# Fil/nd4js

Hardware: AMD Instinct MI355X
Metric: fp64 GFLOP/s: matmul N=4096 & SVD N=2048; % of MFMA/HBM peak (higher is better)
Workload: dtype f64

## Files before the change

nd4js_amd/build.py:

```python
import os
import shutil
import subprocess
import sys
from concurrent.futures import ThreadPoolExecutor

HERE = os.path.dirname(os.path.abspath(__file__))
CSRC = os.path.join(HERE, "csrc")
OBJ = os.path.join(CSRC, "_obj")
LIB = os.path.join(HERE, "libnd4hip.so")
ADDON = os.path.join(HERE, "js", "nd4hip_napi.node")
ARCH = "gfx950"
HIP_SOURCES = ["nd4hip_core.hip", "nd4hip_api.hip", "nd4hip_host.hip", "gemm.hip", "lu.hip", "qr.hip", "svd.hip", "svd_block.hip", "trsm.hip", "chol.hip", "hess.hip", "bidiag.hip", "rrqr.hip"]
HIPCC_FLAGS = ["-O3", "--offload-arch=" + ARCH, "-fPIC", "-std=c++17", "-ffp-contract=on",
               "-mllvm", "-pragma-unroll-threshold=200000", "-Wall", "-Wno-unused-function"]


def _hipcc():
    for c in (os.environ.get("HIPCC"), shutil.which("hipcc"), "/opt/rocm/bin/hipcc"):
        if c and os.path.exists(c):
            return c
    raise RuntimeError("hipcc not found (need ROCm with gfx950 support)")


def _newer(target, deps):
    if not os.path.exists(target):
        return True
    t = os.path.getmtime(target)
    return any(os.path.getmtime(d) > t for d in deps)


def build_lib(force=False, verbose=False):
    os.makedirs(OBJ, exist_ok=True)
    hipcc = _hipcc()
    headers = [os.path.join(CSRC, f) for f in os.listdir(CSRC) if f.endswith(".h")]
    headers.append(os.path.join(HERE, "..", "include", "nd4hip.h"))
    jobs = []
    for s in HIP_SOURCES:
        src = os.path.join(CSRC, s)
        obj = os.path.join(OBJ, s.replace(".hip", ".o"))
        if force or _newer(obj, [src] + headers):
            jobs.append([hipcc] + HIPCC_FLAGS + ["-c", src, "-o", obj])

    def run(cmd):
        if verbose:
            print(" ".join(cmd), flush=True)
        r = subprocess.run(cmd, stdout=subprocess.PIPE, stderr=subprocess.STDOUT, text=True)
        if r.returncode != 0:
            raise RuntimeError("hipcc failed:\n%s\n%s" % (" ".join(cmd), r.stdout))
        if verbose and r.stdout.strip():
            print(r.stdout)
    with ThreadPoolExecutor(max_workers=4) as ex:
        list(ex.map(run, jobs))
    objs = [os.path.join(OBJ, s.replace(".hip", ".o")) for s in HIP_SOURCES]
    if force or jobs or _newer(LIB, objs):
        run([hipcc, "-shared", "-fPIC", "--offload-arch=" + ARCH, "-o", LIB] + objs)
    return LIB


def build_addon(force=False, verbose=False):
    inc = "/usr/include/node"
    src = os.path.join(CSRC, "napi_shim.c")
    if not (os.path.exists(os.path.join(inc, "node_api.h")) and os.path.exists(src)):
        return None
    if force or _newer(ADDON, [src, os.path.join(HERE, "..", "include", "nd4hip.h")]):
        cmd = ["gcc", "-O2", "-fPIC", "-shared", "-std=c11", "-Wall", "-I" + inc, "-I" + os.path.join(HERE, "..", "include"),
# ... 14 lines not shown
```

nd4js_amd/csrc/bidiag.hip:

```cpp
#include "nd4hip_internal.h"
#include "xchg16.h"
#include <cstdio>
#include <cstdlib>

namespace {

constexpr int GR = 8;

__device__ __forceinline__ double blk_max(double v, double* s_red) {
  for (int off = 32; off > 0; off >>= 1) v = fmax(v, __shfl_xor(v, off));
  if ((threadIdx.x & 63) == 0) s_red[threadIdx.x >> 6] = v;
  __syncthreads();
  v = fmax(fmax(s_red[0], s_red[1]), fmax(s_red[2], s_red[3]));
  __syncthreads();
  return v;
}
__device__ __forceinline__ double blk_sum(double v, double* s_red) {
  for (int off = 32; off > 0; off >>= 1) v += __shfl_xor(v, off);
  if ((threadIdx.x & 63) == 0) s_red[threadIdx.x >> 6] = v;
  __syncthreads();
  v = (s_red[0] + s_red[1]) + (s_red[2] + s_red[3]);
  __syncthreads();
  return v;
}
// ... 650 lines not shown
      rq[3] = HpReq{A4r + (unsigned)(t * 2 + 1) * 16, true};
      rq[4] = HpReq{R4p + (unsigned)((q1 * 16 + l1 / E) * V4 + E + l1 % E) * 16, t == 0};
      hp_wait<5>(rs, rq, xv, tag, dead, X.abort, status, delay & 255);
      if (t < T) { s_y[t] = xv[0]; s_cu[t] = xv[1]; }
      if (t == 0) s_alpha = xv[4];
      const double wm = wave_max(xv[2]);
      const double f = wm > 0.0 ? xv[2] * fast_rcp(wm) : 0.0;
      const double wS = wave_sum(xv[3] * f * f);
      if (lane == 0) { s_wm[wave] = wm; s_wS[wave] = wS; }
    }
    if (dead) s_dead = 1;
    __syncthreads();
    if (s_dead) break;
    BP_STAMP(5)
#pragma unroll
    for (int ai = 0; ai < E; ai++) {
      const double ya = s_y[tr + 16 * ai];
#pragma unroll
      for (int bi = 0; bi < E; bi++) a[ai][bi] = fma(-ya, vc[bi], fma(-ur[ai], zc[bi], a[ai][bi]));
    }
    BP_STAMP(6)
  }
#undef BP_STAMP
  if (stamps && t == 0) for (int k = 0; k < 7; k++) stamps[wg * 8 + k] = tacc[k];
}

struct BdWs { double* z; double* y; double* zpart; long sV, sZ; int ncols_total; };

int reflect_left(nd4hip_handle* h, int batch, const Blk& b, const double* A2, long lda, long sA, int acol, const double* tau, long sTau, int tidx, const BdWs& ws) {
  const int nr = b.r1 - b.r0, nc = b.c1 - b.c0;
  if (nr <= 0 || nc <= 0) return 0;
  const int P = (nr + GR - 1) / GR;
  hipLaunchKernelGGL(bd_colsum, dim3((unsigned)((nc + 63) / 64), (unsigned)P, (unsigned)batch), dim3(256), 0, h->stream,
                     b, A2, lda, sA, acol, tau, sTau, tidx, ws.zpart, ws.sZ, ws.ncols_total);
  hipLaunchKernelGGL(bd_colsum_reduce, dim3((unsigned)((nc + 31) / 32), (unsigned)batch), dim3(256), 0, h->stream,
                     b.c0, b.c1, P, ws.zpart, ws.sZ, ws.ncols_total, tau, sTau, tidx, ws.z, ws.sV);
  hipLaunchKernelGGL(bd_rank1, dim3((unsigned)((nc + 255) / 256), (unsigned)((nr + 15) / 16), (unsigned)batch), dim3(256), 0, h->stream,
                     b, A2 + acol, lda, sA, ws.z, ws.sV, tau, sTau, (const int*)nullptr, 0l, tidx);
  ND4_HIP(hipGetLastError());
  return 0;
}
int reflect_right(nd4hip_handle* h, int batch, const Blk& b, const double* v, long sVR, const int* flag, long sF, int fidx, const BdWs& ws) {
  const int nr = b.r1 - b.r0, nc = b.c1 - b.c0;
  if (nr <= 0 || nc <= 0) return 0;
  hipLaunchKernelGGL(bd_rowdot, dim3((unsigned)((nr + 3) / 4), (unsigned)batch), dim3(256), 0, h->stream, b, v, sVR, 2.0, flag, sF, fidx, ws.y, ws.sV);
  hipLaunchKernelGGL(bd_rank1, dim3((unsigned)((nc + 255) / 256), (unsigned)((nr + 15) / 16), (unsigned)batch), dim3(256), 0, h->stream,
                     b, ws.y, 1l, ws.sV, v, sVR, (const double*)nullptr, 0l, flag, sF, fidx);
  ND4_HIP(hipGetLastError());
  return 0;
}

}

int nd4_gebrd(nd4hip_handle* h, int64_t batch64, int64_t M64, int64_t N64, const double* A, double* U, double* B, double* V) {
  ND4_CHECK_ARG(M64 < 32768 && N64 < 32768 && batch64 < 65536, "nd4_gebrd: extent out of range");
  const int M = (int)M64, N = (int)N64, batch = (int)batch64;
  if (M == 0 || N == 0 || batch == 0) return 0;
  const int K = M < N ? M : N, J = M >= N ? K : K + 1;
  const int mx = M > N ? M : N;
  const int Pmax = (M + GR - 1) / GR;
  Nd4WsScope scope(h);
  void* p = nullptr;
  const size_t nd = (size_t)batch * ((size_t)M * N + (size_t)M * K + (size_t)K * N + (size_t)K + 2 * (size_t)mx + (size_t)(Pmax + 24) * mx);
  ND4_TRY(nd4_ws_alloc(h, sizeof(double) * nd + sizeof(int) * (size_t)batch * (2 * (size_t)K + 2) + 256, &p));
  double* W = static_cast<double*>(p);
  double* UL = W + (size_t)batch * M * N;
  double* VR = UL + (size_t)batch * M * K;
  double* tauL = VR + (size_t)batch * K * N;
  BdWs ws;
  ws.z = tauL + (size_t)batch * K; ws.y = ws.z + (size_t)batch * mx; ws.zpart = ws.y + (size_t)batch * mx;
  ws.sV = mx; ws.sZ = (long)Pmax * mx; ws.ncols_total = mx;
  int* flagR = reinterpret_cast<int*>(ws.zpart + (size_t)batch * (Pmax + 24) * mx);
  int* flips = flagR + (size_t)batch * K + 1;
  const long sW = (long)M * N, sUL = (long)M * K, sVRm = (long)K * N;
  ND4_HIP(hipMemcpyAsync(W, A, sizeof(double) * (size_t)batch * sW, hipMemcpyDeviceToDevice, h->stream));
  ND4_HIP(hipMemsetAsync(VR, 0, sizeof(double) * (size_t)batch * sVRm, h->stream));
  ND4_HIP(hipMemsetAsync(flagR, 0, sizeof(int) * (size_t)batch * K, h->stream));

  static const bool fused_off = getenv("ND4HIP_BIDIAG_UNFUSED") != nullptr;
  const bool no_persist = getenv("ND4HIP_BIDIAG_NO_PERSIST") != nullptr;
  bool persist = !fused_off && !no_persist && batch == 1 && M >= 128 && N >= 128 && M <= 2048 && N <= 2048;
  if (persist) {
    int per_cu = 0;
    const hipError_t oe = mx <= 512 ? hipOccupancyMaxActiveBlocksPerMultiprocessor(&per_cu, bdp<2>, 256, 0)
                        : mx <= 1024 ? hipOccupancyMaxActiveBlocksPerMultiprocessor(&per_cu, bdp<4>, 256, 0)
                                     : hipOccupancyMaxActiveBlocksPerMultiprocessor(&per_cu, bdp<8>, 256, 0);
    persist = oe == hipSuccess && (long)per_cu * h->num_cu >= 256;
  }
  if (persist) {
    const int E = mx <= 512 ? 2 : (mx <= 1024 ? 4 : 8), T = 16 * E;
    const size_t V1 = 3 * T, V2 = 2 * E, V3 = T, V4 = 2 * E;
    const size_t xbytes = 16 * 2 * 256 * (V1 + V2 + V3 + V4) + (size_t)BP_NREP * (BP_REP_A2 + BP_REP_A4);
    Nd4WsScope scope2(h);
    void* qp = nullptr;
    ND4_TRY(nd4_ws_alloc(h, sizeof(double) * (size_t)K * M + xbytes + 64, &qp));
    double* ULt = static_cast<double*>(qp);
    BdPx X;
    X.base = reinterpret_cast<qx_u64*>(ULt + (size_t)K * M);
    X.o1 = 0; X.o2 = X.o1 + (unsigned)(2 * 256 * V1 * 16); X.o3 = X.o2 + (unsigned)(2 * 256 * V2 * 16); X.o4 = X.o3 + (unsigned)(2 * 256 * V3 * 16);
    X.oA2 = X.o4 + (unsigned)(2 * 256 * V4 * 16); X.oA4 = X.oA2 + BP_NREP * BP_REP_A2; X.bytes = X.oA4 + BP_NREP * BP_REP_A4;
    X.abort = reinterpret_cast<int*>(reinterpret_cast<char*>(X.base) + xbytes);
    ND4_HIP(hipMemsetAsync(X.base, 0, xbytes + 64, h->stream));
    static const bool want_stamps = getenv("ND4HIP_BDP_STAMPS") != nullptr;
    const int delay = getenv("ND4HIP_BDP_DELAY") ? atoi(getenv("ND4HIP_BDP_DELAY")) : (0 << 8 | 4);
    long long* stamps = nullptr;
    if (want_stamps) { void* sp = nullptr; ND4_TRY(nd4_ws_alloc(h, sizeof(long long) * 256 * 8, &sp)); stamps = static_cast<long long*>(sp); }
    if (E == 2) hipLaunchKernelGGL(bdp<2>, dim3(256), dim3(256), 0, h->stream, W, M, N, K, ULt, tauL, VR, flagR, X, h->xstat, delay, stamps, nd4_test_drop_panel());
// ... 38 lines not shown
      hipLaunchKernelGGL(bd2_finish_row, dim3((unsigned)((N - prev - 1 + 255) / 256)), dim3(256), 0, h->stream, W, N, prev, rowfin);
    ND4_HIP(hipGetLastError());
  } else
  for (int i = 0; i < K; i++) {
    hipLaunchKernelGGL(bd_vec_col, dim3((unsigned)batch), dim3(256), 0, h->stream, W, M, N, i, UL, K, tauL);
    {
      Blk b{W, N, sW, i, M, i + 1, N};
      ND4_TRY(reflect_left(h, batch, b, UL, K, sUL, i, tauL, K, i, ws));
    }
    if (i + 1 < N - 1) {
      hipLaunchKernelGGL(bd_vec_row, dim3((unsigned)batch), dim3(256), 0, h->stream, W, M, N, i, VR, K, flagR);
      Blk b{W, N, sW, i + 1, M, i + 1, N};
      ND4_TRY(reflect_right(h, batch, b, VR + (long)i * N, sVRm, flagR, K, i, ws));
    }
  }
  {
    const unsigned gy = (unsigned)(K < 512 ? K : 512);
    hipLaunchKernelGGL(bd_extract, dim3((unsigned)((J + 255) / 256), gy, (unsigned)batch), dim3(256), 0, h->stream, W, M, N, B, K, J);
  }
  if (batch <= 4 && K >= 256) {
    Nd4WsScope scope2(h);
    void* q = nullptr;
    ND4_TRY(nd4_ws_alloc(h, sizeof(double) * ((size_t)N * K + (size_t)N * J + (size_t)K + 16), &q));
    double* VRt = static_cast<double*>(q);
    double* Vt = VRt + (size_t)N * K;
    double* twos = Vt + (size_t)N * J;
    hipLaunchKernelGGL(bd_fill, dim3((unsigned)((K + 255) / 256)), dim3(256), 0, h->stream, twos, K, 2.0);
    for (int m = 0; m < batch; m++) {
      ND4_TRY(nd4_wy_form(h, M, K, UL + (size_t)m * sUL, tauL + (size_t)m * K, 1, U + (size_t)m * M * K, K));
      ND4_TRY(nd4_transpose(h, K, N, VR + (size_t)m * sVRm, N, VRt, K, 1, 0, 0));
      ND4_TRY(nd4_wy_form(h, N, K, VRt, twos, 1, Vt, J));
      ND4_TRY(nd4_transpose(h, N, J, Vt, J, V + (size_t)m * J * N, N, 1, 0, 0));
    }
  } else {
  {
    const unsigned gy = (unsigned)(M < 512 ? M : 512);
    hipLaunchKernelGGL(bd_set_identity, dim3((unsigned)((K + 255) / 256), gy, (unsigned)batch), dim3(256), 0, h->stream, U, M, K);
  }
  for (int i = K - 1; i >= 0; i--) {
    Blk b{U, K, (long)M * K, i, M, i, K};
    ND4_TRY(reflect_left(h, batch, b, UL, K, sUL, i, tauL, K, i, ws));
  }
  {
    const unsigned gy = (unsigned)(J < 512 ? J : 512);
    hipLaunchKernelGGL(bd_set_identity, dim3((unsigned)((N + 255) / 256), gy, (unsigned)batch), dim3(256), 0, h->stream, V, J, N);
  }
  for (int k = K - 1; k >= 0; k--) {
    if (!(k + 1 < N - 1)) continue;
    Blk b{V, N, (long)J * N, k + 1, J, k + 1, N};
    ND4_TRY(reflect_right(h, batch, b, VR + (long)k * N, sVRm, flagR, K, k, ws));
  }
  }
  ND4_HIP(hipGetLastError());
  return nd4_givens_signs(h, batch, M, K, J, M > N, U, K, (long)M * K, B, J, (long)K * J, tauL, K, flips);
}
```

nd4js_amd/csrc/nd4hip_internal.h:

```cpp
#pragma once
#include <hip/hip_runtime.h>
#include <cstdint>
#include <cstdio>
#include <cstdarg>
#include <vector>
#include "../../include/nd4hip.h"

struct Nd4WsBlock { char* p; size_t size, used; };

struct Nd4Stage { void* p; size_t bytes; bool in_use; };

struct nd4hip_handle {
  int device = 0;
  hipStream_t own_stream = nullptr;
  hipStream_t stream = nullptr;
  std::vector<Nd4WsBlock> ws;
  std::vector<Nd4Stage> stage;
  size_t stage_bytes = 0;
  void* pinned = nullptr;
  size_t pinned_bytes = 0;
  hipEvent_t ev0 = nullptr, ev1 = nullptr;
  hipEvent_t ev_order = nullptr;
  hipStream_t copy_stream = nullptr;
  hipStream_t aux_stream = nullptr;
// ... 15 lines not shown
  }
  ~Nd4DeviceGuard() { if (switched) (void)hipSetDevice(prev); }
  Nd4DeviceGuard(const Nd4DeviceGuard&) = delete;
  Nd4DeviceGuard& operator=(const Nd4DeviceGuard&) = delete;
};

struct Nd4Prof {
  nd4hip_handle* h; bool active;
  Nd4Prof(nd4hip_handle* hh, const char* op, double flops, double bytes);
  ~Nd4Prof();
  Nd4Prof(const Nd4Prof&) = delete;
  Nd4Prof& operator=(const Nd4Prof&) = delete;
};

void nd4_set_error(const char* fmt, ...);
int  nd4_xchg_check(nd4hip_handle* h, const char* where);
int  nd4_test_drop_panel();
int  nd4_hip_fail(hipError_t e, const char* what, const char* file, int line);

#define ND4_HIP(expr)                                                           \
  do { hipError_t _e = (expr);                                                  \
       if (_e != hipSuccess) return nd4_hip_fail(_e, #expr, __FILE__, __LINE__); } while (0)
#define ND4_CHECK_ARG(cond, ...)                                                \
  do { if (!(cond)) { nd4_set_error(__VA_ARGS__); return ND4HIP_ERR_ARG; } } while (0)
#define ND4_TRY(expr) do { int _rc = (expr); if (_rc != 0) return _rc; } while (0)

int nd4_ws_alloc(nd4hip_handle* h, size_t bytes, void** out);
struct Nd4WsScope {
  nd4hip_handle* h; size_t nblocks; size_t used_last; unsigned generation;
  explicit Nd4WsScope(nd4hip_handle* hh);
  ~Nd4WsScope();
};
int nd4_pinned(nd4hip_handle* h, size_t bytes, void** out);

int nd4_gemm(nd4hip_handle* h, bool transA, bool transB, int64_t M, int64_t N, int64_t K,
             double alpha, const double* A, int64_t lda, int64_t sA,
             const double* B, int64_t ldb, int64_t sB,
             double beta, double* C, int64_t ldc, int64_t sC, int64_t batch);

int nd4_getrf(nd4hip_handle* h, int64_t batch, int64_t N, const double* A, double* LU, int32_t* P);
int nd4_getrf_nopivot(nd4hip_handle* h, int64_t batch, int64_t N, const double* A, double* LU, int32_t* P);
int nd4_trsm(nd4hip_handle* h, bool upper, bool unit, int64_t batch, int64_t M, int64_t J, const double* T, int64_t sT, double* X);
int nd4_syrk_lower(nd4hip_handle* h, int64_t N, int64_t K, double alpha, const double* A, int64_t lda, int64_t sA,
                   double beta, double* C, int64_t ldc, int64_t sC, int64_t batch);
int nd4_gemm_nt_lower(nd4hip_handle* h, int64_t N, int64_t K, double alpha, const double* A, int64_t lda, int64_t sA,
                      const double* B, int64_t ldb, int64_t sB, double beta, double* C, int64_t ldc, int64_t sC, int64_t batch);
int nd4_trsm_ld(nd4hip_handle* h, bool upper, bool unit, int64_t batch, int64_t M, int64_t J, const double* T, int64_t ldT, int64_t sT,
                double* X, int64_t sX);
int nd4_trsm_t(nd4hip_handle* h, int64_t batch, int64_t M, int64_t J, const double* T, int64_t ldT, int64_t sT, double* X, int64_t sX);
int nd4_trsm_t_ex(nd4hip_handle* h, bool unit, int64_t batch, int64_t M, int64_t J, const double* T, int64_t ldT, int64_t sT, double* X, int64_t sX);
int nd4_ldltrf(nd4hip_handle* h, int64_t batch, int64_t N, const double* S, double* LD);
int nd4_ldltrs(nd4hip_handle* h, int64_t batch, int64_t N, int64_t J, const double* LD, int64_t sLD, const double* Y, int64_t sY, double* X);
int nd4_gebrd(nd4hip_handle* h, int64_t batch, int64_t M, int64_t N, const double* A, double* U, double* B, double* V);
int nd4_gehrd(nd4hip_handle* h, int64_t batch, int64_t N, const double* A, double* U, double* H);
int nd4_potrf(nd4hip_handle* h, int64_t batch, int64_t N, const double* S, double* L, int* flags);
int nd4_potrs(nd4hip_handle* h, int64_t batch, int64_t N, int64_t J, const double* L, int64_t sL, const double* Y, int64_t sY, double* X);
int nd4_qrls(nd4hip_handle* h, int64_t batch, int64_t N, int64_t M, int64_t I, int64_t J, const double* Q, int64_t sQ,
             const double* R, int64_t sR, const double* Y, int64_t sY, double* X);
int nd4_svdls(nd4hip_handle* h, int64_t batch, int64_t N, int64_t M, int64_t I, int64_t J, const double* U, int64_t sU,
              const double* sv, int64_t sSv, const double* V, int64_t sV, const double* Y, int64_t sY, double* X);
int nd4_getrs(nd4hip_handle* h, int64_t batch, int64_t N, int64_t J, const double* LU, int64_t sLU, const int32_t* P, int64_t sP,
              const double* Y, int64_t sY, double* X);
int nd4_geqrf_q(nd4hip_handle* h, int64_t batch, int64_t M, int64_t N, const double* A, double* Q, double* R);
int nd4_geqr2_panel(nd4hip_handle* h, int batch, int M, double* A, double* V, double* T);
int nd4_givens_signs(nd4hip_handle* h, int batch, int M, int L, int ncols, bool lu_rule, double* Q, long ldq, long sQ,
                     double* R, long ldr, long sR, const double* taus, long sTau, int* flips);
int nd4_wy_form(nd4hip_handle* h, int M, int n, const double* V, const double* Tdiag, int bs, double* Q, int Lq);
int nd4_geqrf_q_ex(nd4hip_handle* h, int64_t batch, int64_t M, int64_t N, const double* A, double* Q, double* R, bool full);
int nd4_geqp3(nd4hip_handle* h, int64_t batch, int64_t M, int64_t N, const double* A, double* Q, double* R, int32_t* P, bool full);
int nd4_qp3rank(nd4hip_handle* h, int64_t batch, int64_t M, int64_t N, const double* R, int64_t sR, int* rank);
int nd4_qp3ls(nd4hip_handle* h, int64_t batch, int64_t N, int64_t M, int64_t I, int64_t J, const double* Q, int64_t sQ,
              const double* R, int64_t sR, const int32_t* P, int64_t sP, const double* Y, int64_t sY, double* X, int* rank_out);
int nd4_gesvdj(nd4hip_handle* h, int64_t batch, int64_t M, int64_t N, const double* A,
               double* U, double* sv, double* V, int* sweeps_out, double* offnorm_out);

int nd4_copy_matrix(nd4hip_handle* h, int64_t rows, int64_t cols, const double* src, int64_t lds,
                    double* dst, int64_t ldd, int64_t batch, int64_t ssrc, int64_t sdst);
int nd4_transpose(nd4hip_handle* h, int64_t rows, int64_t cols, const double* src, int64_t lds,
                  double* dst, int64_t ldd, int64_t batch, int64_t ssrc, int64_t sdst);
int nd4_set_identity(nd4hip_handle* h, int64_t rows, int64_t cols, double* dst, int64_t ldd,
                     int64_t batch, int64_t sdst);
```

nd4js_amd/csrc/svd.hip:

```cpp
#include "svd_internal.h"
#include "dpp.h"
#include <cmath>
#include <cfloat>
#include <cstring>
#include <cstdlib>

namespace {

constexpr int MAX_SWEEPS = 60;

__device__ __forceinline__ double wave_sum(double v) {
#pragma unroll
  for (int off = 32; off > 0; off >>= 1) v += __shfl_xor(v, off);
  return v;
}

__global__ __launch_bounds__(256) void jac_step(double* __restrict__ Wm, double* __restrict__ Utm, int N, long strideM,
                                                 int n2, int step, double tol2, JacState* __restrict__ st,
                                                 const double* __restrict__ floor2, unsigned long long* __restrict__ offmax) {
  const int mat = blockIdx.y;
  if (st[mat].done) return;
  int p, q;
  nd4_rr_pair(n2, step, blockIdx.x, p, q);
  if (q >= N) return;
// ... 378 lines not shown
      }
      if (sweeps >= MAX_SWEEPS) break;
    }
  }
  if (padded) {
    ND4_TRY(nd4_copy_matrix(h, N, N, Wp, Np, W, N, batch, sMp, sM));
    ND4_TRY(nd4_copy_matrix(h, N, N, Utpad, Np, Ut, N, batch, sMp, sM));
  }
  (void)svrp;
  hipLaunchKernelGGL(jac_norms, dim3((unsigned)((N + 3) / 4), (unsigned)batch), dim3(256), 0, h->stream, W, N, sM, svr);
  hipLaunchKernelGGL(jac_rank, dim3((unsigned)((N + 255) / 256), (unsigned)batch), dim3(256), 0, h->stream, svr, N, rank);
  hipLaunchKernelGGL(jac_emit, dim3((unsigned)N, (unsigned)batch), dim3(256), 0, h->stream, W, Ut, N, sM, svr, rank, V, Utp, sv);
  if (N < 128) {
    hipLaunchKernelGGL(jac_complete, dim3((unsigned)batch), dim3(1024), 0, h->stream, V, N, sM, sv, floor2, scratch);
    ND4_HIP(hipGetLastError());
  } else {
    int* z0d = reinterpret_cast<int*>(scratch);
    int* z0h = reinterpret_cast<int*>(static_cast<char*>(pin) + 64);
    hipLaunchKernelGGL(jac_count_rank, dim3((unsigned)((batch + 63) / 64)), dim3(64), 0, h->stream, sv, N, floor2, z0d, batch);
    ND4_HIP(hipGetLastError());
    ND4_HIP(hipMemcpyAsync(z0h, z0d, sizeof(int) * (size_t)batch, hipMemcpyDeviceToHost, h->stream));
    ND4_HIP(hipStreamSynchronize(h->stream));
    for (int m = 0; m < batch; m++) {
      const int r = z0h[m];
      if (r >= N) continue;
      double* Vm = V + (size_t)m * sM;
      if (r == 0) { ND4_TRY(nd4_set_identity(h, N, N, Vm, N, 1, sM)); continue; }
      Nd4WsScope scope3(h);
      void* q = nullptr;
      ND4_TRY(nd4_ws_alloc(h, sizeof(double) * ((size_t)N * N + 2 * (size_t)N * r), &q));
      double* Qf = static_cast<double*>(q);
      double* VrT = Qf + (size_t)N * N;
      double* Rf = VrT + (size_t)N * r;
      ND4_TRY(nd4_transpose(h, r, N, Vm, N, VrT, r, 1, 0, 0));
      ND4_TRY(nd4_geqrf_q_ex(h, 1, N, r, VrT, Qf, Rf, true));
      ND4_TRY(nd4_transpose(h, N, N - r, Qf + r, N, Vm + (size_t)r * N, N, 1, 0, 0));
    }
  }
  ND4_TRY(nd4_transpose(h, N, N, Utp, N, U, N, batch, sM, sM));
  {
    double r; unsigned long long b = last_off; memcpy(&r, &b, 8);
    h->svd_sweeps = sweeps; h->svd_offnorm = sqrt(r); h->svd_rotations = N > 1 ? h_off[1] : 0;
    if (sweeps_out) *sweeps_out = sweeps;
    if (offnorm_out) *offnorm_out = h->svd_offnorm;
  }
  if (sweeps >= MAX_SWEEPS && N > 1) {
    ND4_HIP(hipStreamSynchronize(h->stream));
    nd4_set_error("nd4hip_dgesvdj: no convergence after %d sweeps", sweeps);
    return ND4HIP_ERR_NOCONV;
  }
  return 0;
}

}

int nd4_gesvdj(nd4hip_handle* h, int64_t batch64, int64_t M64, int64_t N64, const double* A,
               double* U, double* sv, double* V, int* sweeps_out, double* offnorm_out) {
  ND4_CHECK_ARG((M64 < N64 ? M64 : N64) < 46000 && M64 < (1ll << 30) && N64 < (1ll << 30) && batch64 < 65536,
                "nd4_gesvdj: extent out of range");
  const int M = (int)M64, N = (int)N64, batch = (int)batch64;
  const int L = M < N ? M : N;
  Nd4WsScope scope(h);
  const long sL = (long)L * L;
  void* p = nullptr;
  if (M == N) {
    ND4_TRY(nd4_ws_alloc(h, sizeof(double) * (size_t)batch * sL, &p));
    double* W = static_cast<double*>(p);
    ND4_HIP(hipMemcpyAsync(W, A, sizeof(double) * (size_t)batch * sL, hipMemcpyDeviceToDevice, h->stream));
    return jacobi_square(h, batch, N, W, U, sv, V, sweeps_out, offnorm_out);
  }
  const long sA = (long)M * N;
  if (M > N) {
    ND4_TRY(nd4_ws_alloc(h, sizeof(double) * (size_t)batch * (sA + 2 * sL), &p));
    double* Q = static_cast<double*>(p); double* R = Q + (size_t)batch * sA; double* Ur = R + (size_t)batch * sL;
    ND4_TRY(nd4_geqrf_q(h, batch, M, N, A, Q, R));
    ND4_TRY(jacobi_square(h, batch, N, R, Ur, sv, V, sweeps_out, offnorm_out));
    return nd4_gemm(h, false, false, M, N, N, 1.0, Q, N, sA, Ur, N, sL, 0.0, U, N, sA, batch);
  }
  ND4_TRY(nd4_ws_alloc(h, sizeof(double) * (size_t)batch * (2 * sA + 3 * sL), &p));
  double* At = static_cast<double*>(p); double* Q = At + (size_t)batch * sA;
  double* R = Q + (size_t)batch * sA; double* Rt = R + (size_t)batch * sL; double* Vr = Rt + (size_t)batch * sL;
  ND4_TRY(nd4_transpose(h, M, N, A, N, At, M, batch, sA, sA));
  ND4_TRY(nd4_geqrf_q(h, batch, N, M, At, Q, R));
  ND4_TRY(nd4_transpose(h, M, M, R, M, Rt, M, batch, sL, sL));
  ND4_TRY(jacobi_square(h, batch, M, Rt, U, sv, Vr, sweeps_out, offnorm_out));
  return nd4_gemm(h, false, true, M, N, M, 1.0, Vr, M, sL, Q, M, sA, 0.0, V, N, sA, batch);
}
```

Measured before the change: 68160.

## Add bidiagonal divide-and-conquer SVD path for single square matrices up to 2048

Adds a new SVD route for batch-1 square matrices with N in (1024, 2048]. It bidiagonalises the matrix, then solves the bidiagonal SVD by divide-and-conquer: Jacobi on small leaves, a secular-equation solve per merge, and GEMM-based back-accumulation of the singular vectors. This replaces one-sided Jacobi sweeps, which need many memory-bound rotation passes over the whole matrix, with mostly GEMM work. It adds a host sync, deflation tolerances that can change accuracy, and a fallback to Jacobi on exchange errors; an environment variable can disable it.

Result: no change. 68140, median of 6 (-0.0%).

```diff
diff --git a/nd4js_amd/build.py b/nd4js_amd/build.py
--- a/nd4js_amd/build.py
+++ b/nd4js_amd/build.py
@@ -10,7 +10,7 @@
 LIB = os.path.join(HERE, "libnd4hip.so")
 ADDON = os.path.join(HERE, "js", "nd4hip_napi.node")
 ARCH = "gfx950"
-HIP_SOURCES = ["nd4hip_core.hip", "nd4hip_api.hip", "nd4hip_host.hip", "gemm.hip", "lu.hip", "qr.hip", "svd.hip", "svd_block.hip", "trsm.hip", "chol.hip", "hess.hip", "bidiag.hip", "rrqr.hip"]
+HIP_SOURCES = ["nd4hip_core.hip", "nd4hip_api.hip", "nd4hip_host.hip", "gemm.hip", "lu.hip", "qr.hip", "svd.hip", "svd_block.hip", "trsm.hip", "chol.hip", "hess.hip", "bidiag.hip", "rrqr.hip", "bdsdc.hip"]
 HIPCC_FLAGS = ["-O3", "--offload-arch=" + ARCH, "-fPIC", "-std=c++17", "-ffp-contract=on",
                "-mllvm", "-pragma-unroll-threshold=200000", "-Wall", "-Wno-unused-function"]
 
diff --git a/nd4js_amd/csrc/bdsdc.hip b/nd4js_amd/csrc/bdsdc.hip
--- /dev/null
+++ b/nd4js_amd/csrc/bdsdc.hip
@@ -0,0 +1,520 @@
+#include "svd_internal.h"
+#include <cmath>
+#include <cfloat>
+#include <cstdlib>
+#include <cstring>
+
+namespace {
+
+constexpr int LEAF_MAX = 32;
+constexpr int LEAF_LD = LEAF_MAX + 1;
+constexpr double EPS = 0x1p-52;
+constexpr double DC_TOL = 16.0 * EPS;
+constexpr int SEC_MAXIT = 100;
+
+__device__ __forceinline__ double wave_sum(double v) {
+#pragma unroll
+  for (int off = 32; off > 0; off >>= 1) v += __shfl_xor(v, off);
+  return v;
+}
+__device__ __forceinline__ double wave_prod(double v) {
+#pragma unroll
+  for (int off = 32; off > 0; off >>= 1) v *= __shfl_xor(v, off);
+  return v;
+}
+
+__global__ __launch_bounds__(1024) void dc_setup(const double* __restrict__ B, int L, int ldb, int np, double* __restrict__ dd,
+                                                 double* __restrict__ ee, double* __restrict__ scale_out) {
+  const int t = threadIdx.x;
+  double mx = 0.0;
+  for (int i = t; i < L; i += 1024) {
+    mx = fmax(mx, fabs(B[(long)i * ldb + i]));
+    if (i + 1 < L) mx = fmax(mx, fabs(B[(long)i * ldb + i + 1]));
+  }
+#pragma unroll
+  for (int off = 32; off > 0; off >>= 1) mx = fmax(mx, __shfl_xor(mx, off));
+  __shared__ double s_mx[16];
+  if ((t & 63) == 0) s_mx[t >> 6] = mx;
+  __syncthreads();
+  mx = 0.0;
+  for (int w = 0; w < 16; w++) mx = fmax(mx, s_mx[w]);
+  int ex = 0;
+  if (mx > 0.0 && isfinite(mx)) { frexp(mx, &ex); }
+  const double sc = ldexp(1.0, -ex);
+  for (int i = t; i < np; i += 1024) {
+    if (i < L) {
+      dd[i] = B[(long)i * ldb + i] * sc;
+      ee[i] = (i + 1 < L) ? B[(long)i * ldb + i + 1] * sc : 0.0;
+    } else {
+      dd[i] = 3.0 + (double)(i - L) * (1.0 / 64.0);
+      ee[i] = 0.0;
+    }
+  }
+  if (t == 0) scale_out[0] = ldexp(1.0, ex);
+}
+
+__global__ __launch_bounds__(256) void dc_leaf(const double* __restrict__ dd, const double* __restrict__ ee, int s, int LD,
+                                               double* __restrict__ U, double* __restrict__ W, double* __restrict__ sig) {
+  __shared__ double s_a[LEAF_LD * LEAF_LD], s_g[LEAF_LD * LEAF_LD], s_u[LEAF_LD * LEAF_LD];
+  __shared__ double s_nrm[LEAF_LD];
+  __shared__ int s_rk[LEAF_LD], s_col[LEAF_LD];
+  __shared__ unsigned s_rot;
+  __shared__ double s_fl;
+  const int t = threadIdx.x, leaf = blockIdx.x;
+  const int r0 = leaf * (s + 1), nc = s + 1;
+  for (int e = t; e < LEAF_LD * LEAF_LD; e += 256) {
+    const int c = e / LEAF_LD, r = e % LEAF_LD;
+    double v = 0.0;
+    if (c < nc && r < s) v = (c == r) ? dd[r0 + r] : ((c == r + 1) ? ee[r0 + r] : 0.0);
+    s_a[e] = v;
+    s_g[e] = (c == r) ? 1.0 : 0.0;
+  }
+  if (t == 0) s_rot = 0;
+  __syncthreads();
+  if (t < nc) {
+    double ss = 0.0;
+    for (int r = 0; r < s; r++) ss += s_a[t * LEAF_LD + r] * s_a[t * LEAF_LD + r];
+    s_nrm[t] = ss;
+  }
+  __syncthreads();
+  const double tol = (double)nc * EPS, tol2 = tol * tol;
+  if (t == 0) { double m = 0.0; for (int c = 0; c < nc; c++) m = fmax(m, s_nrm[c]); s_fl = tol2 * m; }
+  __syncthreads();
+  const double fl = s_fl;
+  const int n2 = (nc + 1) & ~1, pr = t >> 3, sub = t & 7;
+  for (int sweep = 0; sweep < 60; sweep++) {
+    for (int step = 0; step < n2 - 1; step++) {
+      if (pr < n2 / 2) {
+        int p, q;
+        nd4_rr_pair(n2, step, pr, p, q);
+        if (q < nc) {
+          double aa = 0.0, bb = 0.0, ab = 0.0;
+          for (int r = sub; r < s; r += 8) {
+            const double x = s_a[p * LEAF_LD + r], y = s_a[q * LEAF_LD + r];
+            aa += x * x; bb += y * y; ab += x * y;
+          }
+          aa += __shfl_xor(aa, 1); bb += __shfl_xor(bb, 1); ab += __shfl_xor(ab, 1);
+          aa += __shfl_xor(aa, 2); bb += __shfl_xor(bb, 2); ab += __shfl_xor(ab, 2);
+          aa += __shfl_xor(aa, 4); bb += __shfl_xor(bb, 4); ab += __shfl_xor(ab, 4);
+          if (aa > fl && bb > fl && ab * ab > tol2 * aa * bb) {
+            const double zeta = (bb - aa) / (2.0 * ab);
+            const double tn = copysign(1.0, zeta) / (fabs(zeta) + sqrt(1.0 + zeta * zeta));
+            const double c = 1.0 / sqrt(1.0 + tn * tn), sn = c * tn, tau = sn / (1.0 + c);
+            for (int r = sub; r < s; r += 8) {
+              const double x = s_a[p * LEAF_LD + r], y = s_a[q * LEAF_LD + r];
+              s_a[p * LEAF_LD + r] = x - sn * (y + tau * x);
+              s_a[q * LEAF_LD + r] = y + sn * (x - tau * y);
+            }
+            for (int r = sub; r < nc; r += 8) {
+              const double x = s_g[p * LEAF_LD + r], y = s_g[q * LEAF_LD + r];
+              s_g[p * LEAF_LD + r] = x - sn * (y + tau * x);
+              s_g[q * LEAF_LD + r] = y + sn * (x - tau * y);
+            }
+            if (sub == 0) atomicAdd(&s_rot, 1u);
+          }
+        }
+      }
+      __syncthreads();
+    }
+    const unsigned rot = s_rot;
+    __syncthreads();
+    if (t == 0) s_rot = 0;
+    __syncthreads();
+    if (rot == 0) break;
+  }
+  if (t < nc) {
+    double ss = 0.0;
+    for (int r = 0; r < s; r++) ss += s_a[t * LEAF_LD + r] * s_a[t * LEAF_LD + r];
+    s_nrm[t] = ss;
+  }
+  __syncthreads();
+  if (t < nc) {
+    const double x = s_nrm[t];
+    int rk = 0;
+    for (int c = 0; c < nc; c++) rk += (s_nrm[c] > x || (s_nrm[c] == x && c < t)) ? 1 : 0;
+    s_rk[t] = rk;
+    s_col[rk] = t;
+  }
+  __syncthreads();
+  for (int e = t; e < s * s; e += 256) {
+    const int r = e % s, k = e / s, c = s_col[k];
+    const double n2v = s_nrm[c];
+    s_u[k * LEAF_LD + r] = n2v > fl ? s_a[c * LEAF_LD + r] / sqrt(n2v) : 0.0;
+  }
+  __syncthreads();
+  if (t < 64) {
+    for (int k = 0; k < s; k++) {
+      if (s_nrm[s_col[k]] > fl) continue;
+      double w = DBL_MAX;
+      if (t < s) { w = 0.0; for (int j = 0; j < k; j++) w += s_u[j * LEAF_LD + t] * s_u[j * LEAF_LD + t]; }
+      double bw = w; int bi = t;
+#pragma unroll
+      for (int off = 32; off > 0; off >>= 1) {
+        const double ow = __shfl_xor(bw, off); const int oi = __shfl_xor(bi, off);
+        if (ow < bw || (ow == bw && oi < bi)) { bw = ow; bi = oi; }
+      }
+      double v = (t == bi) ? 1.0 : 0.0;
+      for (int pass = 0; pass < 2; pass++) {
+        for (int j = 0; j < k; j++) {
+          const double uj = t < s ? s_u[j * LEAF_LD + t] : 0.0;
+          const double dot = wave_sum(uj * v);
+          v -= dot * uj;
+        }
+      }
+      const double nv = sqrt(wave_sum(v * v));
+      if (t < s) s_u[k * LEAF_LD + t] = v / nv;
+    }
+  }
+  __syncthreads();
+  for (int e = t; e < s * s; e += 256) {
+    const int r = e / s, k = e % s;
+    U[(long)(r0 + r) * LD + r0 + k] = s_u[k * LEAF_LD + r];
+  }
+  for (int e = t; e < nc * nc; e += 256) {
+    const int r = e / nc, k = e % nc;
+    W[(long)(r0 + r) * LD + r0 + k] = s_g[s_col[k] * LEAF_LD + r];
+  }
+  if (t < s) sig[r0 + t] = sqrt(s_nrm[s_col[t]]);
+}
+
+struct DcLevel {
+  int m, nl, nr, LD;
+  const double* dd; const double* ee;
+  const double* sig_in; double* sig_out;
+  double* Win; double* Wout; double* Uout;
+  double* UAt; double* VAt;
+  double* dK; double* zK; int* aK; double* dDf; int* aDf;
+  int* rotp; int* rota; double* rotc; double* rots;
+  int* korg; double* tau; double* sigr; double* zh;
+  int* cnt;
+  unsigned long long* stats;
+  int nreal;
+};
+
+constexpr int PREP_T = 1024;
+constexpr int PREP_SORT = 4096;
+
+__global__ __launch_bounds__(PREP_T) void dc_prep(DcLevel g) {
+  __shared__ double s_key[PREP_SORT];
+  __shared__ unsigned short s_idx[PREP_SORT];
+  __shared__ double s_z[PREP_SORT / 2 + 64];
+  __shared__ int s_nd;
+  const int t = threadIdx.x, q = blockIdx.x;
+  const int N = g.m, nl = g.nl, nr = g.nr, LD = g.LD;
+  const int r0 = q * (N + 1), k = r0 + nl, r1 = r0 + N;
+  const double alpha = g.dd[k], beta = g.ee[k];
+  const double lam1 = g.Win[(long)k * LD + k];
+  const double lam2 = g.Win[(long)(k + 1) * LD + r1];
+  const double za = alpha * lam1, zb = beta * lam2;
+  const double z0 = hypot(za, zb);
+  const double c0 = z0 > 0.0 ? za / z0 : 1.0, s0 = z0 > 0.0 ? zb / z0 : 0.0;
+  int P = 1;
+  while (P < N) P <<= 1;
+  for (int a = t; a < P; a += PREP_T) {
+    double d = INFINITY;
+    if (a < nl) { d = g.sig_in[r0 + a]; s_z[a] = alpha * g.Win[(long)k * LD + r0 + a]; }
+    else if (a == nl) { d = 0.0; s_z[a] = z0; }
+    else if (a < N) { d = g.sig_in[k + 1 + (a - nl - 1)]; s_z[a] = beta * g.Win[(long)(k + 1) * LD + k + 1 + (a - nl - 1)]; }
+    s_key[a] = d; s_idx[a] = (unsigned short)a;
+  }
+  __syncthreads();
+  for (int r = r0 + t; r <= r1; r += PREP_T) {
+    if (r <= k) { const double x = g.Win[(long)r * LD + k]; g.Wout[(long)r * LD + r1] = -s0 * x; g.Win[(long)r * LD + k] = c0 * x; }
+    else { const double x = g.Win[(long)r * LD + r1]; g.Wout[(long)r * LD + r1] = c0 * x; g.Win[(long)r * LD + r1] = s0 * x; }
+  }
+  for (int len = 2; len <= P; len <<= 1) {
+    for (int j = len >> 1; j > 0; j >>= 1) {
+      for (int i = t; i < P; i += PREP_T) {
+        const int l = i ^ j;
+        if (l > i) {
+          const double ki = s_key[i], kl = s_key[l];
+          const int ii = s_idx[i], il = s_idx[l];
+          const bool gt = ki > kl || (ki == kl && (il == nl || (ii != nl && ii > il)));
+          const bool up = (i & len) == 0;
+          if (gt == up) { s_key[i] = kl; s_key[l] = ki; s_idx[i] = (unsigned short)il; s_idx[l] = (unsigned short)ii; }
+        }
+      }
+      __syncthreads();
+    }
+  }
+  if (t == 0) {
+    const double tol = DC_TOL;
+    double* dK = g.dK + r0; double* zK = g.zK + r0; int* aK = g.aK + r0;
+    int* rp = g.rotp + r0; int* ra = g.rota + r0; double* rc = g.rotc + r0; double* rs = g.rots + r0;
+    double zmid = s_z[nl];
+    if (fabs(zmid) <= tol) zmid = tol;
+    dK[0] = 0.0; zK[0] = zmid; aK[0] = nl;
+    int K = 1, nd = 0, nrot = 0;
+    int pa = -1; double pd = 0.0, pz = 0.0;
+    for (int pos = 1; pos < N; pos++) {
+      const int a = s_idx[pos]; const double da = s_key[pos]; const double za = s_z[a];
+      if (fabs(za) <= tol) { s_key[nd] = da; s_idx[nd] = (unsigned short)a; nd++; continue; }
+      if (pa >= 0 && da - pd <= tol) {
+        const double r = hypot(pz, za), c = za / r, sn = pz / r;
+        rp[nrot] = pa; ra[nrot] = a; rc[nrot] = c; rs[nrot] = sn; nrot++;
+        int i = nd;
+        while (i > 0 && s_key[i - 1] > pd) { s_key[i] = s_key[i - 1]; s_idx[i] = s_idx[i - 1]; i--; }
+        s_key[i] = pd; s_idx[i] = (unsigned short)pa; nd++;
+        pa = a; pd = da; pz = r;
+        continue;
+      }
+      if (pa >= 0) { dK[K] = pd; zK[K] = pz; aK[K] = pa; K++; }
+      pa = a; pd = da; pz = za;
+    }
+    if (pa >= 0) { dK[K] = pd; zK[K] = pz; aK[K] = pa; K++; }
+    if (K > 1 && dK[1] < 0.5 * tol) dK[1] = 0.5 * tol;
+    g.cnt[4 * q] = K; g.cnt[4 * q + 1] = nd; g.cnt[4 * q + 2] = nrot;
+    s_nd = nd;
+  }
+  __syncthreads();
+  const int nd = s_nd;
+  for (int i = t; i < nd; i += PREP_T) { g.dDf[r0 + i] = s_key[i]; g.aDf[r0 + i] = s_idx[i]; }
+}
+
+__device__ __forceinline__ void sec_eval(const double* __restrict__ dk, const double* __restrict__ zk, int K, double d0, double tau,
+                                         double& f, double& g) {
+  const int lane = threadIdx.x & 63;
+  double fs = 0.0, gs = 0.0;
+  for (int j = lane; j < K; j += 64) {
+    const double dj = dk[j];
+    const double den = ((dj - d0) - tau) * (dj + d0 + tau);
+    const double zz = zk[j] * zk[j];
+    const double tj = zz / den;
+    fs += tj; gs += tj / den;
+  }
+  f = 1.0 + wave_sum(fs);
+  g = wave_sum(gs);
+}
+
+__global__ __launch_bounds__(256) void dc_secular(DcLevel g) {
+  const int q = blockIdx.y, r0 = q * (g.m + 1);
+  const int K = g.cnt[4 * q];
+  const int i = blockIdx.x * 4 + (threadIdx.x >> 6);
+  if (i >= K) return;
+  const double* dk = g.dK + r0; const double* zk = g.zK + r0;
+  int org; double lo, hi, tau;
+  unsigned evals = 0;
+  double f, gd;
+  if (i < K - 1) {
+    const double dl = dk[i], half = 0.5 * (dk[i + 1] - dl);
+    sec_eval(dk, zk, K, dl, half, f, gd); evals++;
+    if (f >= 0.0) { org = i; lo = 0.0; hi = half; }
+    else { org = i + 1; lo = -half; hi = 0.0; }
+    tau = 0.5 * (lo + hi);
+  } else {
+    const int lane = threadIdx.x & 63;
+    double zz = 0.0;
+    for (int j = lane; j < K; j += 64) zz += zk[j] * zk[j];
+    zz = wave_sum(zz);
+    const double dl = dk[i];
+    org = i; lo = 0.0; hi = zz / (sqrt(dl * dl + zz) + dl);
+    tau = 0.5 * hi;
+  }
+  const double d0 = dk[org];
+  for (int it = 0; it < SEC_MAXIT; it++) {
+    sec_eval(dk, zk, K, d0, tau, f, gd); evals++;
+    if (f == 0.0) break;
+    if (f < 0.0) lo = tau; else hi = tau;
+    const double del = -tau * (2.0 * d0 + tau);
+    const double am = f - gd * del;
+    const double dn = -gd * del * del / am;
+    const double r2 = d0 * d0 - dn;
+    double tn = -dn / (d0 + sqrt(r2));
+    if (!(tn > lo && tn < hi)) tn = 0.5 * (lo + hi);
+    const bool done = fabs(tn - tau) <= 2.0 * EPS * fabs(tn) || (hi - lo) <= 2.0 * EPS * fmax(fabs(lo), fabs(hi));
+    tau = tn;
+    if (done) break;
+  }
+  if ((threadIdx.x & 63) == 0) {
+    g.korg[r0 + i] = org; g.tau[r0 + i] = tau; g.sigr[r0 + i] = d0 + tau;
+    atomicAdd(&g.stats[0], (unsigned long long)evals);
+    atomicMax(&g.stats[1], (unsigned long long)evals);
+  }
+}
+
+__global__ __launch_bounds__(256) void dc_zhat(DcLevel g) {
+  const int q = blockIdx.y, r0 = q * (g.m + 1);
+  const int K = g.cnt[4 * q];
+  const int j = blockIdx.x * 4 + (threadIdx.x >> 6), lane = threadIdx.x & 63;
+  if (j >= K) return;
+  const double* dk = g.dK + r0;
+  const double dj = dk[j];
+  double p = 1.0;
+  for (int i = lane; i < K; i += 64) {
+    const double dko = dk[g.korg[r0 + i]], ti = g.tau[r0 + i];
+    const double num = ((dko - dj) + ti) * (dko + ti + dj);
+    if (i == K - 1) p *= num;
+    else if (i < j) p *= num / ((dk[i] - dj) * (dk[i] + dj));
+    else p *= num / ((dk[i + 1] - dj) * (dk[i + 1] + dj));
+  }
+  p = wave_prod(p);
+  if (lane == 0) g.zh[r0 + j] = copysign(sqrt(fabs(p)), g.zK[r0 + j]);
+}
+
+__global__ __launch_bounds__(256) void dc_vectors(DcLevel g) {
+  __shared__ double s_u[PREP_SORT / 2 + 64], s_v[PREP_SORT / 2 + 64];
+  __shared__ int s_jof[PREP_SORT / 2 + 64];
+  __shared__ double s_red[8];
+  const int q = blockIdx.y, x = blockIdx.x, t = threadIdx.x;
+  const int N = g.m, nl = g.nl, LD = g.LD;
+  const int r0 = q * (N + 1), k = r0 + nl;
+  const int K = g.cnt[4 * q], nd = g.cnt[4 * q + 1];
+  const double* dk = g.dK + r0;
+  double sval; int rank;
+  double nu = 1.0, nv = 1.0;
+  int adefl = -1;
+  if (x < K) {
+    for (int a = t; a < N; a += 256) s_jof[a] = -1;
+    __syncthreads();
+    for (int j = t; j < K; j += 256) s_jof[g.aK[r0 + j]] = j;
+    const int org = g.korg[r0 + x];
+    const double d0 = dk[org], tau = g.tau[r0 + x];
+    sval = d0 + tau;
+    double su = 0.0, sv = 0.0;
+    for (int j = t; j < K; j += 256) {
+      const double dj = dk[j];
+      const double den = ((dj - d0) - tau) * (dj + d0 + tau);
+      const double v = g.zh[r0 + j] / den;
+      const double u = j == 0 ? -1.0 : dj * v;
+      s_v[j] = v; s_u[j] = u;
+      su += u * u; sv += v * v;
+    }
+    su = wave_sum(su); sv = wave_sum(sv);
+    if ((t & 63) == 0) { s_red[t >> 6] = su; s_red[4 + (t >> 6)] = sv; }
+    __syncthreads();
+    nu = 1.0 / sqrt((s_red[0] + s_red[1]) + (s_red[2] + s_red[3]));
+    nv = 1.0 / sqrt((s_red[4] + s_red[5]) + (s_red[6] + s_red[7]));
+    int lo = 0, hi = nd;
+    while (lo < hi) { const int mid = (lo + hi) >> 1; if (g.dDf[r0 + mid] < sval) lo = mid + 1; else hi = mid; }
+    rank = x + lo;
+  } else {
+    const int m = x - K;
+    sval = g.dDf[r0 + m]; adefl = g.aDf[r0 + m];
+    int lo = 0, hi = K;
+    while (lo < hi) { const int mid = (lo + hi) >> 1; if (g.sigr[r0 + mid] <= sval) lo = mid + 1; else hi = mid; }
+    rank = m + lo;
+  }
+  if (g.nreal > 0 && rank < g.nreal) rank = g.nreal - 1 - rank;
+  double* urow = g.UAt + (long)(r0 + rank) * LD + r0;
+  double* vrow = g.VAt + (long)(r0 + rank) * LD + r0;
+  if (x < K) {
+    for (int a = t; a <= N; a += 256) {
+      const int j = a < N ? s_jof[a] : 0;
+      urow[a] = (a < N && j >= 0) ? s_u[j] * nu : 0.0;
+      vrow[a] = j >= 0 ? s_v[j] * nv : 0.0;
+    }
+    if (t == 0) { g.Uout[(long)k * LD + r0 + rank] = -nu; g.sig_out[r0 + rank] = sval; }
+  } else {
+    for (int a = t; a <= N; a += 256) { const double e = a == adefl ? 1.0 : 0.0; urow[a] = e; vrow[a] = e; }
+    if (t == 0) { g.Uout[(long)k * LD + r0 + rank] = 0.0; g.sig_out[r0 + rank] = sval; }
+  }
+}
+
+__global__ __launch_bounds__(256) void dc_rotate(DcLevel g) {
+  const int q = blockIdx.x, N = g.m, LD = g.LD, r0 = q * (N + 1);
+  const int nrot = g.cnt[4 * q + 2];
+  if (nrot == 0) return;
+  for (int r = threadIdx.x; r < N; r += 256) {
+    double* ur = g.UAt + (long)(r0 + r) * LD + r0;
+    double* vr = g.VAt + (long)(r0 + r) * LD + r0;
+    for (int i = nrot - 1; i >= 0; i--) {
+      const int p = g.rotp[r0 + i], a = g.rota[r0 + i];
+      const double c = g.rotc[r0 + i], s = g.rots[r0 + i];
+      double x = ur[p], y = ur[a];
+      ur[p] = c * x + s * y; ur[a] = -s * x + c * y;
+      x = vr[p]; y = vr[a];
+      vr[p] = c * x + s * y; vr[a] = -s * x + c * y;
+    }
+  }
+}
+
+__global__ void dc_zero_ucols(double* __restrict__ U, int m, int nl, int LD) {
+  const int q = blockIdx.y, r0 = q * (m + 1), k = r0 + nl, r1 = r0 + m;
+  const int r = r0 + blockIdx.x * blockDim.x + threadIdx.x;
+  if (r >= r1 || r == k) return;
+  U[(long)r * LD + (r < k ? k : r1)] = 0.0;
+}
+
+__global__ void dc_finish(const double* __restrict__ sig, const double* __restrict__ scale, int L, double* __restrict__ sv) {
+  const int i = blockIdx.x * blockDim.x + threadIdx.x;
+  if (i < L) sv[i] = sig[i] * scale[0];
+}
+
+}
+
+int nd4_bdsdc_svd(nd4hip_handle* h, int L, const double* Ubd, const double* B, const double* Vbd, double* U, double* sv, double* V) {
+  ND4_CHECK_ARG(L >= 2 && L <= 4096, "nd4_bdsdc_svd: L = %d out of range", L);
+  int D = 0;
+  while (((L + 1) + (1 << D) - 1) / (1 << D) > LEAF_MAX + 1) D++;
+  const int s = ((L + 1) + (1 << D) - 1) / (1 << D) - 1;
+  const int np = (1 << D) * (s + 1) - 1, LD = np + 1;
+  ND4_CHECK_ARG(np < PREP_SORT / 2 + 64, "nd4_bdsdc_svd: padded size %d too large", np);
+  Nd4WsScope scope(h);
+  const size_t sq = (size_t)LD * LD;
+  const size_t nvec = 12;
+  void* p = nullptr;
+  ND4_TRY(nd4_ws_alloc(h, sizeof(double) * (6 * sq + 4 * (size_t)LD + nvec * (size_t)LD + 64) + sizeof(int) * (4 * (size_t)LD + 64) + 256, &p));
+  double* Ub[2] = {static_cast<double*>(p), static_cast<double*>(p) + sq};
+  double* Wb[2] = {Ub[1] + sq, Ub[1] + 2 * sq};
+  double* UAt = Wb[1] + sq;
+  double* VAt = UAt + sq;
+  double* sg[2] = {VAt + sq, VAt + sq + LD};
+  double* dd = sg[1] + LD;
+  double* ee = dd + LD;
+  double* lists = ee + LD;
+  double* scale = lists + nvec * (size_t)LD;
+  unsigned long long* stats = reinterpret_cast<unsigned long long*>(scale + 8);
+  int* cnt = reinterpret_cast<int*>(scale + 64);
+  DcLevel g;
+  g.dK = lists; g.zK = lists + LD; g.dDf = lists + 2 * LD; g.rotc = lists + 3 * LD; g.rots = lists + 4 * LD;
+  g.tau = lists + 5 * LD; g.sigr = lists + 6 * LD; g.zh = lists + 7 * LD;
+  int* il = reinterpret_cast<int*>(lists + 8 * LD);
+  g.aK = il; g.aDf = il + LD; g.rotp = il + 2 * LD; g.rota = il + 3 * LD; g.korg = il + 4 * LD;
+  g.cnt = cnt; g.LD = LD; g.dd = dd; g.ee = ee;
+  ND4_HIP(hipMemsetAsync(scale, 0, sizeof(double) * 64, h->stream));
+  hipLaunchKernelGGL(dc_setup, dim3(1), dim3(1024), 0, h->stream, B, L, L, np, dd, ee, scale);
+  hipLaunchKernelGGL(dc_leaf, dim3(1u << D), dim3(256), 0, h->stream, dd, ee, s, LD, Ub[0], Wb[0], sg[0]);
+  ND4_HIP(hipGetLastError());
+  int cur = 0;
+  for (int d = D - 1; d >= 0; d--) {
+    const int m = (1 << (D - d)) * (s + 1) - 1, nl = (m - 1) / 2, nr = m - 1 - nl, Q = 1 << d;
+    g.m = m; g.nl = nl; g.nr = nr;
+    g.sig_in = sg[cur]; g.sig_out = sg[cur ^ 1];
+    g.Win = Wb[cur]; g.Wout = Wb[cur ^ 1]; g.Uout = Ub[cur ^ 1];
+    g.UAt = UAt; g.VAt = VAt;
+    g.stats = stats + 2 * d;
+    g.nreal = d == 0 ? L : 0;
+    hipLaunchKernelGGL(dc_prep, dim3((unsigned)Q), dim3(PREP_T), 0, h->stream, g);
+    hipLaunchKernelGGL(dc_secular, dim3((unsigned)((m + 3) / 4), (unsigned)Q), dim3(256), 0, h->stream, g);
+    hipLaunchKernelGGL(dc_zhat, dim3((unsigned)((m + 3) / 4), (unsigned)Q), dim3(256), 0, h->stream, g);
+    hipLaunchKernelGGL(dc_vectors, dim3((unsigned)m, (unsigned)Q), dim3(256), 0, h->stream, g);
+    hipLaunchKernelGGL(dc_rotate, dim3((unsigned)Q), dim3(256), 0, h->stream, g);
+    hipLaunchKernelGGL(dc_zero_ucols, dim3((unsigned)((m + 255) / 256), (unsigned)Q), dim3(256), 0, h->stream, Ub[cur], m, nl, LD);
+    ND4_HIP(hipGetLastError());
+    const long S = (long)(m + 1) * (LD + 1);
+    const long top = 0, bot = (long)(nl + 1) * (LD + 1);
+    ND4_TRY(nd4_gemm(h, false, true, nl, m, nl + 1, 1.0, Ub[cur] + top, LD, S, UAt, LD, S, 0.0, Ub[cur ^ 1], LD, S, Q));
+    ND4_TRY(nd4_gemm(h, false, true, nr, m, nr + 1, 1.0, Ub[cur] + bot, LD, S, UAt + (nl + 1), LD, S, 0.0,
+                     Ub[cur ^ 1] + (long)(nl + 1) * LD, LD, S, Q));
+    ND4_TRY(nd4_gemm(h, false, true, nl + 1, m, nl + 1, 1.0, Wb[cur] + top, LD, S, VAt, LD, S, 0.0, Wb[cur ^ 1], LD, S, Q));
+    ND4_TRY(nd4_gemm(h, false, true, nr + 1, m, nr + 1, 1.0, Wb[cur] + bot, LD, S, VAt + (nl + 1), LD, S, 0.0,
+                     Wb[cur ^ 1] + (long)(nl + 1) * LD, LD, S, Q));
+    cur ^= 1;
+  }
+  ND4_TRY(nd4_gemm(h, false, false, L, L, L, 1.0, Ubd, L, 0, Ub[cur], LD, 0, 0.0, U, L, 0, 1));
+  ND4_TRY(nd4_gemm(h, true, false, L, L, L, 1.0, Wb[cur], LD, 0, Vbd, L, 0, 0.0, V, L, 0, 1));
+  hipLaunchKernelGGL(dc_finish, dim3((unsigned)((L + 255) / 256)), dim3(256), 0, h->stream, sg[cur], scale, L, sv);
+  ND4_HIP(hipGetLastError());
+  static const bool stats_on = getenv("ND4HIP_DC_STATS") != nullptr;
+  if (stats_on) {
+    unsigned long long hs[48];
+    ND4_HIP(hipMemcpyAsync(hs, stats, sizeof(unsigned long long) * 2 * D, hipMemcpyDeviceToHost, h->stream));
+    ND4_HIP(hipStreamSynchronize(h->stream));
+    for (int d = 0; d < D; d++) {
+      const int m = (1 << (D - d)) * (s + 1) - 1;
+      fprintf(stderr, "[nd4hip bdsdc] L=%d n'=%d leaf %d: level %d (%d merges of %d): secular evaluations %llu, max per root %llu\n",
+              L, np, s, d, 1 << d, m, hs[2 * d], hs[2 * d + 1]);
+    }
+  }
+  return 0;
+}
diff --git a/nd4js_amd/csrc/bidiag.hip b/nd4js_amd/csrc/bidiag.hip
--- a/nd4js_amd/csrc/bidiag.hip
+++ b/nd4js_amd/csrc/bidiag.hip
@@ -726,7 +726,7 @@
 
 }
 
-int nd4_gebrd(nd4hip_handle* h, int64_t batch64, int64_t M64, int64_t N64, const double* A, double* U, double* B, double* V) {
+int nd4_gebrd_ex(nd4hip_handle* h, int64_t batch64, int64_t M64, int64_t N64, const double* A, double* U, double* B, double* V, bool ref_signs) {
   ND4_CHECK_ARG(M64 < 32768 && N64 < 32768 && batch64 < 65536, "nd4_gebrd: extent out of range");
   const int M = (int)M64, N = (int)N64, batch = (int)batch64;
   if (M == 0 || N == 0 || batch == 0) return 0;
@@ -871,5 +871,10 @@
   }
   }
   ND4_HIP(hipGetLastError());
+  if (!ref_signs) return 0;
   return nd4_givens_signs(h, batch, M, K, J, M > N, U, K, (long)M * K, B, J, (long)K * J, tauL, K, flips);
 }
+
+int nd4_gebrd(nd4hip_handle* h, int64_t batch, int64_t M, int64_t N, const double* A, double* U, double* B, double* V) {
+  return nd4_gebrd_ex(h, batch, M, N, A, U, B, V, true);
+}
diff --git a/nd4js_amd/csrc/nd4hip_internal.h b/nd4js_amd/csrc/nd4hip_internal.h
--- a/nd4js_amd/csrc/nd4hip_internal.h
+++ b/nd4js_amd/csrc/nd4hip_internal.h
@@ -91,6 +91,8 @@
 int nd4_ldltrf(nd4hip_handle* h, int64_t batch, int64_t N, const double* S, double* LD);
 int nd4_ldltrs(nd4hip_handle* h, int64_t batch, int64_t N, int64_t J, const double* LD, int64_t sLD, const double* Y, int64_t sY, double* X);
 int nd4_gebrd(nd4hip_handle* h, int64_t batch, int64_t M, int64_t N, const double* A, double* U, double* B, double* V);
+int nd4_gebrd_ex(nd4hip_handle* h, int64_t batch, int64_t M, int64_t N, const double* A, double* U, double* B, double* V, bool ref_signs);
+int nd4_bdsdc_svd(nd4hip_handle* h, int L, const double* Ubd, const double* B, const double* Vbd, double* U, double* sv, double* V);
 int nd4_gehrd(nd4hip_handle* h, int64_t batch, int64_t N, const double* A, double* U, double* H);
 int nd4_potrf(nd4hip_handle* h, int64_t batch, int64_t N, const double* S, double* L, int* flags);
 int nd4_potrs(nd4hip_handle* h, int64_t batch, int64_t N, int64_t J, const double* L, int64_t sL, const double* Y, int64_t sY, double* X);
diff --git a/nd4js_amd/csrc/svd.hip b/nd4js_amd/csrc/svd.hip
--- a/nd4js_amd/csrc/svd.hip
+++ b/nd4js_amd/csrc/svd.hip
@@ -454,6 +454,34 @@
   return 0;
 }
 
+int dc_square(nd4hip_handle* h, int N, const double* W, double* U, double* sv, double* V, int* sweeps_out, double* offnorm_out) {
+  Nd4WsScope scope(h);
+  const size_t sq = (size_t)N * N;
+  void* p = nullptr;
+  ND4_TRY(nd4_ws_alloc(h, sizeof(double) * 3 * sq, &p));
+  double* Ubd = static_cast<double*>(p);
+  double* Bd = Ubd + sq;
+  double* Vbd = Bd + sq;
+  ND4_TRY(nd4_gebrd_ex(h, 1, N, N, W, Ubd, Bd, Vbd, false));
+  ND4_HIP(hipStreamSynchronize(h->stream));
+  ND4_TRY(nd4_xchg_check(h, "nd4hip_dgesvdj (bidiagonalisation)"));
+  ND4_TRY(nd4_bdsdc_svd(h, N, Ubd, Bd, Vbd, U, sv, V));
+  h->svd_sweeps = 0; h->svd_rotations = 0; h->svd_offnorm = 0.0;
+  if (sweeps_out) *sweeps_out = 0;
+  if (offnorm_out) *offnorm_out = 0.0;
+  return 0;
+}
+
+int square_svd(nd4hip_handle* h, int batch, int N, double* W, double* U, double* sv, double* V, int* sweeps_out, double* offnorm_out) {
+  const char* dc_env = getenv("ND4HIP_SVD_DC");
+  const bool dc_off = dc_env != nullptr && dc_env[0] == '0';
+  if (!dc_off && batch == 1 && N > 1024 && N <= 2048) {
+    const int rc = dc_square(h, N, W, U, sv, V, sweeps_out, offnorm_out);
+    if (rc != ND4HIP_ERR_XCHG) return rc;
+  }
+  return jacobi_square(h, batch, N, W, U, sv, V, sweeps_out, offnorm_out);
+}
+
 }
 
 int nd4_gesvdj(nd4hip_handle* h, int64_t batch64, int64_t M64, int64_t N64, const double* A,
@@ -469,14 +497,14 @@
     ND4_TRY(nd4_ws_alloc(h, sizeof(double) * (size_t)batch * sL, &p));
     double* W = static_cast<double*>(p);
     ND4_HIP(hipMemcpyAsync(W, A, sizeof(double) * (size_t)batch * sL, hipMemcpyDeviceToDevice, h->stream));
-    return jacobi_square(h, batch, N, W, U, sv, V, sweeps_out, offnorm_out);
+    return square_svd(h, batch, N, W, U, sv, V, sweeps_out, offnorm_out);
   }
   const long sA = (long)M * N;
   if (M > N) {
     ND4_TRY(nd4_ws_alloc(h, sizeof(double) * (size_t)batch * (sA + 2 * sL), &p));
     double* Q = static_cast<double*>(p); double* R = Q + (size_t)batch * sA; double* Ur = R + (size_t)batch * sL;
     ND4_TRY(nd4_geqrf_q(h, batch, M, N, A, Q, R));
-    ND4_TRY(jacobi_square(h, batch, N, R, Ur, sv, V, sweeps_out, offnorm_out));
+    ND4_TRY(square_svd(h, batch, N, R, Ur, sv, V, sweeps_out, offnorm_out));
     return nd4_gemm(h, false, false, M, N, N, 1.0, Q, N, sA, Ur, N, sL, 0.0, U, N, sA, batch);
   }
   ND4_TRY(nd4_ws_alloc(h, sizeof(double) * (size_t)batch * (2 * sA + 3 * sL), &p));
@@ -485,6 +513,6 @@
   ND4_TRY(nd4_transpose(h, M, N, A, N, At, M, batch, sA, sA));
   ND4_TRY(nd4_geqrf_q(h, batch, N, M, At, Q, R));
   ND4_TRY(nd4_transpose(h, M, M, R, M, Rt, M, batch, sL, sL));
-  ND4_TRY(jacobi_square(h, batch, M, Rt, U, sv, Vr, sweeps_out, offnorm_out));
+  ND4_TRY(square_svd(h, batch, M, Rt, U, sv, Vr, sweeps_out, offnorm_out));
   return nd4_gemm(h, false, true, M, N, M, 1.0, Vr, M, sL, Q, M, sA, 0.0, V, N, sA, batch);
 }
```
